# NTT123/vietTTS

Hardware: AMD Instinct MI355X
Metric: audio samples/sec whole-node, HiFi-GAN V1 mel2wave (higher is better)
Workload: dtype bf16; 1 GPU; HiFi-GAN V1 generator, 64 utterances x 1024 mel frames per GPU per step (BASELINE configs[2] shape), bf16; batch_per_gpu=64, frames=1024, parallelism=dp1 utterance-sharded, weights broadcast once, no data-path collective, microbatch=0, streams=0, schedule=engine default: micro-batches of <= 32768 frames on two HIP streams

## Files before the change

viettts_amd/csrc/kernels_bf16_rbg.hip:

```cpp
#include <stdio.h>
#include <string.h>

#include <type_traits>
#include <utility>

#include "bf16_common.h"

namespace vtts {

template <class F, int... I>
__device__ __forceinline__ void static_for(std::integer_sequence<int, I...>, F&& f) {
    (f(std::integral_constant<int, I>{}), ...);
}

constexpr int XCD_MAP_MIN_TILES = 192;

template <int C_, int KS_, int N1_, int WM_, int WN_, int PA_, int MINWG_, int XC_ = C_, int BLK_ = 32>
struct GTile {
    static constexpr int C = C_, KS = KS_, N1 = N1_, WM = WM_, WN = WN_, PA = PA_, MINWG = MINWG_, BLK = BLK_;
    static constexpr int XC = XC_, NXC = C / XC;
    static constexpr int MR16 = C / WM / 16, NR16 = N1 / WN / 16, NH = NR16 / 4;
    static constexpr int KS32 = C / 32, KSX32 = XC / 32;
        static constexpr int LA16 = 3, RA16 = LA16 + 1;
    static_assert(BLK == 32 || BLK == 16, "MFMA block shape");
    static_assert(BLK == 32 || (XC >= 64 && C / WM == 64 && (N1 / WN) % 64 == 0 && (KSX32 % 4 == 0 || (NXC == 1 && 4 % KSX32 == 0)) && 4 % RA16 == 0), "16-block tiles: C >= 64, 64-row wave tiles");
    static constexpr int THREADS = 64 * WM * WN;
    static constexpr int MR = C / WM / 32, NR = N1 / WN / 32;
    static constexpr int H2 = (KS - 1) / 2;
    static constexpr int MAXDIL = 5;
    static constexpr int NT2 = N1 - 2 * H2;
    static constexpr int SPR1 = XC / 8, P1 = XC * 2;
    static constexpr int SPR2 = C / 8, P2 = C * 2;
    static constexpr int ROWSX_MAX = N1 + 2 * H2 * MAXDIL;
    static constexpr int ROWST = N1 + 2 * H2;
    static constexpr int KSTEPS = C / 16;
    static constexpr int KSX = XC / 16;
    static constexpr int NQT = KS * KSTEPS;
    static constexpr int MB = C / 32;
    static constexpr int RA = PA + 1;
    static constexpr bool UNROLL_ALL = (KSX % RA) != 0;
    static constexpr bool WREG = UNROLL_ALL && NXC == 1 && NQT * MR * 4 <= 96;
    static constexpr int XPT = (ROWSX_MAX * SPR1 + THREADS - 1) / THREADS;
    static constexpr size_t CONV_BYTES = (size_t)KS * C * C * 2;
    static_assert(C % (WM * 32) == 0 && N1 % (WN * 32) == 0, "tile/wave mismatch");
    static_assert(C % XC == 0 && (NXC == 1 || !UNROLL_ALL), "channel chunking");
    static_assert(SPR1 == 4 || SPR1 == 8 || SPR1 == 16, "X row pitch 64..256 B");
    static_assert(SPR2 == 4 || SPR2 == 8 || SPR2 == 16 || SPR2 == 32, "xt row pitch 64..512 B");
    static constexpr bool RAWRES = NXC == 1 && C == 32;
    static constexpr int RAW_BYTES = RAWRES ? tile_rows16(N1) * P1 : 0;
    static __host__ __device__ constexpr int tile_bytes(int dil) {
        const int bx = tile_rows16(N1 + 2 * H2 * dil) * P1, bt = tile_rows16(ROWST) * P2;
        return bx > bt ? bx : bt;
    }
    static constexpr bool TAIL = false;
    static constexpr int TAIL_KS = 7, TAIL_H = 3;
    static constexpr int TAIL_BYTES = 0;
    static constexpr bool UP = false;
    static constexpr int OH = 0;
    static int lds_bytes(int dil) { return tile_bytes(dil) + RAW_BYTES; }
    static_assert(tile_rows16(ROWSX_MAX) * P1 + RAW_BYTES <= 80 * 1024 || !RAWRES, "two workgroups per CU");
    static_assert(tile_rows16(ROWSX_MAX) * P1 <= 160 * 1024 && tile_rows16(ROWST) * P2 <= 160 * 1024, "LDS budget");
};

template <class B>
struct GTail : B {
    static constexpr bool TAIL = true;
    static constexpr int TAIL_BYTES = 1024;
    static constexpr int OH = B::TAIL_H;
    static int lds_bytes(int dil) { return B::tile_bytes(dil) + B::RAW_BYTES + TAIL_BYTES; }
    static_assert(B::RAWRES && B::C == 32 && B::WM == 1, "the tail lives on the C = 32 tile with the LDS-resident residual rows");
    static_assert(B::tile_bytes(B::MAXDIL) + B::RAW_BYTES + TAIL_BYTES <= 80 * 1024, "two workgroups per CU");
};

template <class B>
struct GUp : B {
    static constexpr bool UP = true;
    static constexpr int OH = 1;
    static constexpr int UWN = B::WM * B::WN;
    static constexpr int UNR = B::N1 / UWN / 32;
    static constexpr int UMR = B::C / 2 / 32;
    static constexpr int UKS = B::C / 16;
    static constexpr int UP_BYTES = 3 * B::C * B::C * 2;
    static_assert(B::BLK == 16 && !B::RAWRES && !B::TAIL && B::NXC == 1 && (B::C == 128 || B::C == 64), "the stage-ending k = 11 classes (both run 16-blocks)");
    static_assert(B::N1 % (UWN * 32) == 0 && UMR >= 1 && UKS % 2 == 0, "whole 32 x 32 blocks");
    static_assert(B::N1 + 2 <= B::ROWST, "frames t0 - 1 .. t0 + N1 fit the xt tile");
    static_assert(B::tile_bytes(B::MAXDIL) <= 80 * 1024, "two workgroups per CU");
};

template <class T>
__global__ __launch_bounds__(T::THREADS, (T::MINWG * T::THREADS + 255) / 256) void resblock_pair_g_bf16_k(BConvArgs a) {
    constexpr int C = T::C, KS = T::KS, N1 = T::N1, WN = T::WN, PA = T::PA, RA = T::RA;
    constexpr int THREADS = T::THREADS, MR = T::MR, NR = T::NR, H2 = T::H2, NT2 = T::NT2;
    constexpr int SPR1 = T::SPR1, P1 = T::P1, SPR2 = T::SPR2, P2 = T::P2, XC = T::XC, NXC = T::NXC, KSX = T::KSX;
    constexpr int KSTEPS = T::KSTEPS, NQT = T::NQT, MB = T::MB, XPT = T::XPT;
    constexpr int BLK = T::BLK;
    constexpr bool B16 = BLK == 16;
    constexpr int MR16 = T::MR16, NR16 = T::NR16, NH = T::NH;
    static_assert(!B16 || (!T::RAWRES && !T::TAIL && !T::WREG && !T::UNROLL_ALL), "16-block tiles are the rolled-loop C >= 64 tiles");

    extern __shared__ __attribute__((aligned(16))) unsigned char lds[];
    unsigned char* xt = lds;
    [[maybe_unused]] unsigned char* const xraw = lds + (T::RAWRES ? T::tile_bytes(a.dil) : 0);

    const int tid = threadIdx.x;
    const int lane = tid & 63;
    const int wave = tid >> 6;
    const int wm = wave / WN;
    const int wn = wave % WN;
    const int l31 = lane & 31;
    const int lh = lane >> 5;
    const int l15 = lane & 15;
    const int lg = lane >> 4;
    const int b = a.zrev ? (int)(gridDim.z - 1 - blockIdx.z) : (int)blockIdx.z;
    const int Lp = a.L;
    const int L = a.lens ? min(max(a.lens[b], 0) * a.len_mul, a.L) : a.L;
    constexpr int OH = T::OH, TS = NT2 - 2 * OH;
    const bool xmap = (a.L + TS - 1) / TS >= XCD_MAP_MIN_TILES;
    const int nt = (L + TS - 1) / TS, r = (int)((blockIdx.x + b) & 7), lo = (r * nt) >> 3, hi = ((r + 1) * nt) >> 3;
    const int tile = xmap ? lo + (int)(blockIdx.x >> 3) : (int)blockIdx.x;
    if (xmap && tile >= hi) return;
    const int t0 = tile * TS - OH;
    if (t0 + OH >= L) return;
    const int dil = a.dil;
    const int h1 = H2 * dil;
    const int rowsx = N1 + 2 * h1;
    const unsigned short* __restrict__ xg = static_cast<const unsigned short*>(a.x) + (size_t)b * Lp * C;
    [[maybe_unused]] const int wg_lin = blockIdx.z * gridDim.x + blockIdx.x;
    VTTS_TL_ID(a, wg_lin);
    VTTS_TL(a, wg_lin, 0);

    typedef float f32x4 __attribute__((ext_vector_type(4)));
    f32x16 acc[B16 ? 1 : MR][B16 ? 1 : NR];
    f32x16 bblk[B16 ? 1 : MR];
    f32x4 acc16[B16 ? MR16 : 1][B16 ? NR16 : 1];
    f32x4 bblk16[B16 ? MR16 : 1];
    auto load_bias = [&](const float* __restrict__ bias) {
        typedef float f32x8 __attribute__((ext_vector_type(8)));
        if constexpr (B16) {
#pragma unroll
            for (int mr = 0; mr < MR16; ++mr) bblk16[mr] = *reinterpret_cast<const f32x4*>(bias + wm * (C / T::WM) + mr * 16 + 4 * lg);
            return;
        }
#pragma unroll
        for (int mr = 0; mr < MR; ++mr) {
            const float* __restrict__ bp = bias + wm * (C / T::WM) + mr * 32 + 4 * lh;
            const f32x4 q0 = *reinterpret_cast<const f32x4*>(bp), q1 = *reinterpret_cast<const f32x4*>(bp + 8);
            const f32x4 q2 = *reinterpret_cast<const f32x4*>(bp + 16), q3 = *reinterpret_cast<const f32x4*>(bp + 24);
            const f32x8 lo = __builtin_shufflevector(q0, q1, 0, 1, 2, 3, 4, 5, 6, 7), hi = __builtin_shufflevector(q2, q3, 0, 1, 2, 3, 4, 5, 6, 7);
            bblk[mr] = __builtin_shufflevector(lo, hi, 0, 1, 2, 3, 4, 5, 6, 7, 8, 9, 10, 11, 12, 13, 14, 15);
        }
    };
    load_bias(a.bias);
    if constexpr (T::TAIL) {
        float* tw = reinterpret_cast<float*>(lds + T::tile_bytes(dil) + T::RAW_BYTES);
        for (int i = tid; i < T::TAIL_KS * C; i += THREADS) tw[i] = a.tail_wf[i];
    }

    constexpr int NQW = T::WREG ? NQT : 1;
    bf16x8 aw[NQW][MR];
    auto load_w_all = [&](const unsigned char* __restrict__ wconv) {
        if constexpr (T::WREG) {
            const uint4* __restrict__ ap = reinterpret_cast<const uint4*>(wconv) + (size_t)(wm * MR) * 64 + lane;
#pragma unroll
            for (int q = 0; q < NQT; ++q)
#pragma unroll
                for (int mr = 0; mr < MR; ++mr) aw[q][mr] = __builtin_bit_cast(bf16x8, ap[(size_t)(q * MB + mr) * 64]);
        }
    };
    load_w_all(static_cast<const unsigned char*>(a.wp));

    auto stage_x = [&](int xc, auto xb_tag) {
        constexpr int XB = decltype(xb_tag)::value;
        constexpr int RPI = THREADS / SPR1;
        static_assert(THREADS % SPR1 == 0 && RPI % 16 == 0, "a thread's units share their column and their swizzle");
        const int tx0 = t0 - H2 - h1;
        constexpr int RW = 64 / SPR1;
        const int row0 = SPR1 >= 16 ? tid / SPR1 : wave * RW + lane % RW, c = SPR1 >= 16 ? tid % SPR1 : lane / RW;
        auto act2 = [](unsigned u) { return lrelu01_pack(bf16_lo(u), bf16_hi(u)); };
        unsigned char* const lds0 = xt + tile_off<SPR1, BLK>(row0, c);
        [[maybe_unused]] auto keep_raw = [&](int r, int cc, const uint4& raw, bool live) {
            const int rr = r - H2 - h1;
            if (live && rr >= 0 && rr < N1) *reinterpret_cast<uint4*>(xraw + tile_off<SPR1, BLK>(rr, cc)) = raw;
        };
        if (tx0 >= 0 && tx0 + XPT * RPI <= L) {
            const unsigned short* __restrict__ g0 = xg + (size_t)(tx0 + row0) * C + xc * XC + c * 8;
#pragma unroll
            for (int i0 = 0; i0 < XPT; i0 += XB) {
                uint4 v[XB];
#pragma unroll
                for (int i = 0; i < XB; ++i)
                    if (i0 + i < XPT) v[i] = *reinterpret_cast<const uint4*>(g0 + (size_t)(i0 + i) * RPI * C);
#if VTTS_TIMELINE
                if (i0 == 0) {
                    VTTS_TL(a, wg_lin, 7);
                    __builtin_amdgcn_s_waitcnt(0x0f70);
                    VTTS_TL(a, wg_lin, 8);
                }
#endif
                if constexpr (T::RAWRES) {
#pragma unroll
                    for (int i = 0; i < XB; ++i) keep_raw(row0 + (i0 + i) * RPI, c, v[i], i0 + i < XPT);
                }
#pragma unroll
                for (int i = 0; i < XB; ++i) {
                    v[i].x = act2(v[i].x);
                    v[i].y = act2(v[i].y);
                    v[i].z = act2(v[i].z);
                    v[i].w = act2(v[i].w);
                }
#pragma unroll
                for (int i = 0; i < XB; ++i)
                    if (i0 + i < XPT && row0 + (i0 + i) * RPI < rowsx) *reinterpret_cast<uint4*>(lds0 + (i0 + i) * RPI * P1) = v[i];
            }
            return;
        }
#pragma unroll
        for (int i0 = 0; i0 < XPT; i0 += XB) {
            uint4 v[XB];
            bool okx[XB];
#pragma unroll
            for (int i = 0; i < XB; ++i) {
                const int t = tx0 + row0 + (i0 + i) * RPI;
                okx[i] = i0 + i < XPT && row0 + (i0 + i) * RPI < rowsx && t >= 0 && t < L;
                const int tc = t < 0 ? 0 : (t >= L ? L - 1 : t);
                v[i] = *reinterpret_cast<const uint4*>(xg + (size_t)tc * C + xc * XC + c * 8);
            }
#pragma unroll
            for (int i = 0; i < XB; ++i) {
                if (!okx[i]) v[i] = make_uint4(0u, 0u, 0u, 0u);
                if constexpr (T::RAWRES) keep_raw(row0 + (i0 + i) * RPI, c, v[i], i0 + i < XPT);
                v[i].x = act2(v[i].x);
                v[i].y = act2(v[i].y);
                v[i].z = act2(v[i].z);
                v[i].w = act2(v[i].w);
            }
#pragma unroll
            for (int i = 0; i < XB; ++i)
                if (i0 + i < XPT && row0 + (i0 + i) * RPI < rowsx) *reinterpret_cast<uint4*>(lds0 + (i0 + i) * RPI * P1) = v[i];
        }
    };
    stage_x(0, std::integral_constant<int, XPT>{});
    VTTS_TL(a, wg_lin, 9);
    __syncthreads();
    VTTS_TL(a, wg_lin, 1);

    const int rowbase0 = wn * (N1 / WN) + l31;
    auto conv_phase = [&](const unsigned char* __restrict__ wconv, int dl, auto sprb_tag, auto nks_tag, int ks0, auto fresh_tag) {
        constexpr int SPRB = decltype(sprb_tag)::value, PB = SPRB * 16, NKS = decltype(nks_tag)::value;
        constexpr bool FRESH = decltype(fresh_tag)::value;
        constexpr int NSTEPS = KS * NKS;
        const uint4* __restrict__ aptr = reinterpret_cast<const uint4*>(wconv) + ((size_t)ks0 * MB + wm * MR) * 64 + lane;
        bf16x8 af[RA][MR], bf[2][NR];
        auto load_a = [&](int tap, int ks, int slot) {
            const int tc = tap < KS ? tap : KS - 1;
#pragma unroll
            for (int mr = 0; mr < MR; ++mr)
                af[slot][mr] = __builtin_bit_cast(bf16x8, aptr[(size_t)((tc * KSTEPS + ks) * MB + mr) * 64]);
        };
        auto load_b = [&](int tap, int ks, int par) {
#pragma unroll
            for (int nr = 0; nr < NR; ++nr) {
                const int row = rowbase0 + tap * dl + nr * 32;
                bf[par][nr] = *reinterpret_cast<const bf16x8*>(xt + tile_off<SPRB, BLK>(row, ks * 2 + lh));
            }
        };
        auto mfma_step = [&](int slot, int par, bool first) {
#pragma unroll
            for (int mr = 0; mr < MR; ++mr)
#pragma unroll
                for (int nr = 0; nr < NR; ++nr) {
                    acc[mr][nr] = __builtin_amdgcn_mfma_f32_32x32x16_bf16(af[slot][mr], bf[par][nr], first ? bblk[mr] : acc[mr][nr], 0, 0, 0);

                }
        };
        auto pin_step = [&](bool has_b) {
            constexpr int NM = MR * NR;
            const int mem = MR + (has_b ? NR : 0);
            int done = 0;
            for (int i = 0; i < NM; ++i) {
                __builtin_amdgcn_sched_group_barrier(0x008, 1, 0);
                const int upto = (i + 1) * mem / NM;
                for (; done < upto; ++done) {
                    if (done < MR) __builtin_amdgcn_sched_group_barrier(0x020, 1, 0);
                    else __builtin_amdgcn_sched_group_barrier(0x100, 1, 0);
                }
            }
        };
        static_assert(T::UNROLL_ALL || PA <= NKS, "look-ahead within two taps");
#pragma unroll
        for (int s = 0; s < PA; ++s) load_a(s / NKS, s % NKS, s % RA);
        load_b(0, 0, 0);
        __builtin_amdgcn_sched_group_barrier(0x020, MR * PA, 0);
        __builtin_amdgcn_sched_group_barrier(0x100, NR, 0);
        if constexpr (T::UNROLL_ALL) {
#pragma unroll
            for (int s = 0; s < NSTEPS; ++s) {
                load_a((s + PA) / NKS, (s + PA) % NKS, (s + PA) % RA);
                if (s + 1 < NSTEPS) load_b((s + 1) / NKS, (s + 1) % NKS, (s + 1) & 1);
                mfma_step(s % RA, s & 1, FRESH && s == 0);
                pin_step(s + 1 < NSTEPS);
            }
        } else {
            constexpr int UB = NKS < 8 ? NKS : 8;
            static_assert(T::UNROLL_ALL || (UB % RA == 0 && UB % 2 == 0 && NKS % UB == 0), "ring slot / B parity must be compile-time in the block loop");
            typedef unsigned u32x4_t __attribute__((ext_vector_type(4)));
            const auto rs_w = __builtin_amdgcn_make_buffer_rsrc(const_cast<unsigned char*>(wconv), 0, (int)T::CONV_BYTES, 0x00020000);
            const unsigned a_voff = (unsigned)((wm * MR) * 64 + lane) * 16;
            auto load_a2 = [&](int sa, int slot) {
                const int sc = sa < NSTEPS ? sa : NSTEPS - 1;
                const int tap = sc / NKS, ks = sc - tap * NKS;
                const int soff = ((tap * KSTEPS + ks0 + ks) * MB) * 1024;
#pragma unroll
                for (int mr = 0; mr < MR; ++mr) {
                    const u32x4_t v = __builtin_amdgcn_raw_buffer_load_b128(rs_w, a_voff + mr * 1024, soff, 0);
                    af[slot][mr] = __builtin_bit_cast(bf16x8, v);
                }
            };
            auto tap_terms = [&](int tap, unsigned& tapaddr, unsigned& xs) {
                const int row = rowbase0 + tap * dl;
                if constexpr (SPRB >= 16) {
                    tapaddr = (unsigned)row * PB;
                    xs = (unsigned)(swz_of<SPRB>(row) ^ lh) << 4;
                } else {
                    tapaddr = (unsigned)tile_off<SPRB, BLK>(row, lh);
                    xs = 0;
                }
            };
            auto load_b2 = [&](unsigned tapaddr, unsigned xs, int ks, int par) {
                const unsigned addr = SPRB >= 16 ? tapaddr + (xs ^ (unsigned)(ks << 5)) : tapaddr + (unsigned)(ks << 9);
#pragma unroll
                for (int nr = 0; nr < NR; ++nr) bf[par][nr] = *reinterpret_cast<const bf16x8*>(xt + addr + nr * 32 * PB);
            };
            auto block = [&](int s0, auto first_tag) {
                const int tap = s0 / NKS, ksb = s0 - tap * NKS;
                unsigned ta, xs, tn, xn;
                tap_terms(tap, ta, xs);
                const bool wrap = ksb + UB >= NKS;
                const int tapn = tap + 1 < KS ? tap + 1 : KS - 1;
                tap_terms(wrap ? tapn : tap, tn, xn);
                const int ksn = wrap ? 0 : ksb + UB;
#pragma unroll
                for (int i = 0; i < UB; ++i) {
                    load_a2(s0 + i + PA, (i + PA) % RA);
                    if (i + 1 < UB) load_b2(ta, xs, ksb + i + 1, (i + 1) & 1);
                    else load_b2(tn, xn, ksn, (i + 1) & 1);
                    mfma_step(i % RA, i & 1, decltype(first_tag)::value && i == 0);
                    pin_step(true);
                }
            };
            block(0, std::integral_constant<bool, FRESH>{});
#pragma nounroll
            for (int s0 = UB; s0 < NSTEPS; s0 += UB) block(s0, std::false_type{});
        }
    };

    auto conv_phase_wreg = [&](int dl, auto sprb_tag) {
        constexpr int SPRB = decltype(sprb_tag)::value;
        bf16x8 bf[2][NR];
        auto load_b = [&](int q, int par) {
            const int tap = q / KSTEPS, ks = q % KSTEPS;
#pragma unroll
            for (int nr = 0; nr < NR; ++nr) bf[par][nr] = *reinterpret_cast<const bf16x8*>(xt + tile_off<SPRB, BLK>(rowbase0 + tap * dl + nr * 32, ks * 2 + lh));
        };
        load_b(0, 0);
        __builtin_amdgcn_sched_group_barrier(0x100, NR, 0);
#pragma unroll
        for (int q = 0; q < NQT; ++q) {
            if (q + 1 < NQT) load_b(q + 1, (q + 1) & 1);
#pragma unroll
            for (int mr = 0; mr < MR; ++mr)
#pragma unroll
                for (int nr = 0; nr < NR; ++nr)
                    acc[mr][nr] = __builtin_amdgcn_mfma_f32_32x32x16_bf16(aw[q < NQW ? q : 0][mr], bf[q & 1][nr], q == 0 ? bblk[mr] : acc[mr][nr], 0, 0, 0);
            for (int i = 0; i < MR * NR; ++i) {
                __builtin_amdgcn_sched_group_barrier(0x008, 1, 0);
                if (q + 1 < NQT && i < NR) __builtin_amdgcn_sched_group_barrier(0x100, 1, 0);
            }
        }
    };


    const int rowbase16 = wn * (N1 / WN) + l15;
    auto conv_phase16 = [&](const unsigned char* __restrict__ wconv, int dl, auto sprb_tag, auto nks_tag, int ks0, auto fresh_tag) {
        constexpr int SPRB = decltype(sprb_tag)::value, PB = SPRB * 16, NKS = decltype(nks_tag)::value;
        constexpr bool FRESH = decltype(fresh_tag)::value;
        constexpr int NSTEPS = KS * NKS, LA = T::LA16, RA = T::RA16, UB = 4, APU = MR16 / NH;
        constexpr int REM = NSTEPS % UB;
        static_assert((NKS % UB == 0 || UB % NKS == 0) && UB % RA == 0 && (UB * NH) % 2 == 0, "ring slot / B parity must be compile-time in the block loop");
        const auto rs_w = __builtin_amdgcn_make_buffer_rsrc(const_cast<unsigned char*>(wconv), 0, (int)T::CONV_BYTES, 0x00020000);
        const unsigned a_voff = (unsigned)((wm * MR16) * 64 + lane) * 16;
        bf16x8 af[RA][MR16], bf[2][4];
        auto load_a = [&](int sa, auto h_tag, auto slot_tag) {
            constexpr int h = decltype(h_tag)::value, slot = decltype(slot_tag)::value;
            const int sc = sa < NSTEPS ? sa : NSTEPS - 1;
            const int tap = sc / NKS, ks = sc - tap * NKS;
            const int soff = ((tap * T::KS32 + ks0 + ks) * (C / 16)) * 1024;
#pragma unroll
            for (int m = h * APU; m < (h + 1) * APU; ++m) af[slot][m] = __builtin_bit_cast(bf16x8, __builtin_amdgcn_raw_buffer_load_b128(rs_w, a_voff + m * 1024, soff, 0));
        };
        auto tap_terms = [&](int tap, unsigned& tapaddr, unsigned& xs) {
            const int row = rowbase16 + tap * dl;
            if constexpr (SPRB >= 16) {
                tapaddr = (unsigned)row * PB;
                xs = (unsigned)(swz_of<SPRB, 16>(row) ^ lg) << 4;
            } else {
                tapaddr = (unsigned)tile_off<SPRB, BLK>(row, lg);
                xs = 0;
            }
        };
        auto load_b = [&](unsigned tapaddr, unsigned xs, int ks, int h, auto par_tag) {
            const unsigned addr = SPRB >= 16 ? tapaddr + (xs ^ (unsigned)(ks << 6)) : tapaddr + (unsigned)(ks << 10);
#pragma unroll
            for (int nr = 0; nr < 4; ++nr) bf[decltype(par_tag)::value][nr] = *reinterpret_cast<const bf16x8*>(xt + addr + (4 * h + nr) * 16 * PB);
        };
        auto pin_unit = [&](auto nds_tag, auto nvm_tag) {
            constexpr int NDS = decltype(nds_tag)::value, NVM = decltype(nvm_tag)::value;
            int done = 0;
#pragma unroll
            for (int i = 0; i < 16; ++i) {
                __builtin_amdgcn_sched_group_barrier(0x008, 1, 0);
                const int upto = (i + 1) * (NDS + NVM) / 16;
#pragma unroll
                for (; done < upto; ++done) {
                    if (done < NDS) __builtin_amdgcn_sched_group_barrier(0x100, 1, 0);
                    else __builtin_amdgcn_sched_group_barrier(0x020, 1, 0);
                }
            }
        };
        unsigned ta0, xs0;
        tap_terms(0, ta0, xs0);
        static_for(std::make_integer_sequence<int, LA * NH>{}, [&](auto v) {
            constexpr int s = decltype(v)::value / NH, h = decltype(v)::value % NH;
            load_a(s, std::integral_constant<int, h>{}, std::integral_constant<int, s % RA>{});
        });
        load_b(ta0, xs0, 0, 0, std::integral_constant<int, 0>{});
        __builtin_amdgcn_sched_group_barrier(0x020, MR16 * LA, 0);
        __builtin_amdgcn_sched_group_barrier(0x100, 4, 0);
        auto block = [&](int s0, auto nu_tag) {
            constexpr int NU = decltype(nu_tag)::value, NT = NKS >= UB ? 1 : (NU + NKS - 1) / NKS;
            constexpr bool PEEL = NU < UB;
            const int tap = s0 / NKS, ksb = s0 - tap * NKS;
            unsigned ta[NT], xs[NT], tn, xn;
#pragma unroll
            for (int t = 0; t < NT; ++t) tap_terms(tap + t, ta[t], xs[t]);
            const bool wrap = ksb + UB >= NKS;
            const int tapn = tap + NT < KS ? tap + NT : KS - 1;
            tap_terms(wrap ? tapn : tap, tn, xn);
            const int ksn = wrap ? 0 : ksb + UB;
            static_for(std::make_integer_sequence<int, NU * NH>{}, [&](auto v) {
                constexpr int u = decltype(v)::value, i = u / NH, h = u % NH;
                constexpr int ti = NKS >= UB ? 0 : i / NKS, ki = i - ti * NKS;
                constexpr int tj = NKS >= UB ? 0 : (i + 1) / NKS, kj = i + 1 - tj * NKS;
                constexpr bool last = h + 1 == NH && i + 1 == NU;
                if constexpr (!PEEL) load_a(s0 + i + LA, std::integral_constant<int, h>{}, std::integral_constant<int, (i + LA) % RA>{});
                constexpr auto par = std::integral_constant<int, (u + 1) & 1>{};
                if constexpr (h + 1 < NH) load_b(ta[ti], xs[ti], ksb + ki, h + 1, par);
                else if constexpr (i + 1 < NU) load_b(ta[tj], xs[tj], ksb + kj, 0, par);
                else if constexpr (!PEEL) load_b(tn, xn, ksn, 0, par);
#pragma unroll
                for (int nr = 0; nr < 4; ++nr)
#pragma unroll
                    for (int mr = 0; mr < MR16; ++mr)
                        acc16[mr][4 * h + nr] = __builtin_amdgcn_mfma_f32_16x16x32_bf16(af[i % RA][mr], bf[u & 1][nr], acc16[mr][4 * h + nr], 0, 0, 0);
                pin_unit(std::integral_constant<int, PEEL && last ? 0 : 4>{}, std::integral_constant<int, PEEL ? 0 : APU>{});
            });
        };
        if constexpr (FRESH) {
#pragma unroll
            for (int mr = 0; mr < MR16; ++mr)
#pragma unroll
                for (int nr = 0; nr < NR16; ++nr) acc16[mr][nr] = bblk16[mr];
        }
#pragma nounroll
        for (int s0 = 0; s0 < NSTEPS - REM; s0 += UB) block(s0, std::integral_constant<int, UB>{});
        if constexpr (REM != 0) block(NSTEPS - REM, std::integral_constant<int, REM>{});
    };

#pragma unroll
    for (int xc = 0; xc < NXC; ++xc) {
        if (xc > 0) {
            __syncthreads();
            stage_x(xc, std::integral_constant<int, 4>{});
            __syncthreads();
        }
        if constexpr (B16) {
            if (xc == 0) conv_phase16(static_cast<const unsigned char*>(a.wp), dil, std::integral_constant<int, SPR1>{}, std::integral_constant<int, T::KSX32>{}, 0, std::true_type{});
            else conv_phase16(static_cast<const unsigned char*>(a.wp), dil, std::integral_constant<int, SPR1>{}, std::integral_constant<int, T::KSX32>{}, xc * T::KSX32, std::false_type{});
        } else if constexpr (T::WREG)
            conv_phase_wreg(dil, std::integral_constant<int, SPR1>{});
        else if (xc == 0)
            conv_phase(static_cast<const unsigned char*>(a.wp), dil, std::integral_constant<int, SPR1>{}, std::integral_constant<int, KSX>{}, 0, std::true_type{});
        else
            conv_phase(static_cast<const unsigned char*>(a.wp), dil, std::integral_constant<int, SPR1>{}, std::integral_constant<int, KSX>{}, xc * KSX, std::false_type{});
    }
    VTTS_TL(a, wg_lin, 2);
    load_w_all(static_cast<const unsigned char*>(a.wp) + T::CONV_BYTES);
    __syncthreads();


    load_bias(a.bias + C);
    [[maybe_unused]] const int col16 = wn * (N1 / WN) + 16 * (lg & 1) + l15;
    {
        if constexpr (B16) {
#pragma unroll
            for (int mr = 0; mr < MR16; ++mr) {
                const int cb = wm * (C / T::WM) + mr * 16;
#pragma unroll
                for (int j = 0; j < NR16 / 2; ++j) {
                    const int tp = t0 - H2 + wn * (N1 / WN) + 32 * j + l15, tq = tp + 16;
                    unsigned p0 = lrelu01_pack(acc16[mr][2 * j][0], acc16[mr][2 * j][1]);
                    unsigned p1 = lrelu01_pack(acc16[mr][2 * j][2], acc16[mr][2 * j][3]);
                    unsigned q0 = lrelu01_pack(acc16[mr][2 * j + 1][0], acc16[mr][2 * j + 1][1]);
                    unsigned q1 = lrelu01_pack(acc16[mr][2 * j + 1][2], acc16[mr][2 * j + 1][3]);
                    if (!(tp >= 0 && tp < L)) p0 = p1 = 0u;
                    if (!(tq >= 0 && tq < L)) q0 = q1 = 0u;
                    swap_pair16(p0, q0);
                    swap_pair16(p1, q1);
                    *reinterpret_cast<uint4*>(xt + tile_off<SPR2, BLK>(col16 + 32 * j, (cb >> 3) + (lg >> 1))) = make_uint4(p0, p1, q0, q1);
                }
            }
        } else {
#pragma unroll
        for (int mr = 0; mr < MR; ++mr) {
#pragma unroll
            for (int p = 0; p < 2; ++p) {
                const int cb = wm * (C / T::WM) + mr * 32 + 16 * p;
#pragma unroll
                for (int nr = 0; nr < NR; ++nr) {
                    const int row = wn * (N1 / WN) + nr * 32 + l31;
                    const int tt = t0 - H2 + row;
                    const bool ok = tt >= 0 && tt < L;
                    const int r0 = 8 * p;
                    unsigned p0 = lrelu01_pack(acc[mr][nr][r0 + 0], acc[mr][nr][r0 + 1]);
                    unsigned p1 = lrelu01_pack(acc[mr][nr][r0 + 2], acc[mr][nr][r0 + 3]);
                    unsigned q0 = lrelu01_pack(acc[mr][nr][r0 + 4], acc[mr][nr][r0 + 5]);
                    unsigned q1 = lrelu01_pack(acc[mr][nr][r0 + 6], acc[mr][nr][r0 + 7]);
                    if (!ok) p0 = p1 = q0 = q1 = 0u;
                    swap_pair(p0, q0);
                    swap_pair(p1, q1);
                    const int slot = (cb >> 3) + lh;
                    *reinterpret_cast<uint4*>(xt + tile_off<SPR2, BLK>(row, slot)) = make_uint4(p0, p1, q0, q1);
                }
            }
        }
        }
        for (int u = tid; u < 2 * H2 * SPR2; u += THREADS) {
            const int row = N1 + u % (2 * H2), c = u / (2 * H2);
            *reinterpret_cast<uint4*>(xt + tile_off<SPR2, BLK>(row, c)) = make_uint4(0u, 0u, 0u, 0u);
        }
    }
    __syncthreads();
    VTTS_TL(a, wg_lin, 3);

    if constexpr (B16)
        conv_phase16(static_cast<const unsigned char*>(a.wp) + T::CONV_BYTES, 1, std::integral_constant<int, SPR2>{}, std::integral_constant<int, T::KS32>{}, 0, std::true_type{});
    else if constexpr (T::WREG)
        conv_phase_wreg(1, std::integral_constant<int, SPR2>{});
    else
        conv_phase(static_cast<const unsigned char*>(a.wp) + T::CONV_BYTES, 1, std::integral_constant<int, SPR2>{}, std::integral_constant<int, KSTEPS>{}, 0, std::true_type{});
    VTTS_TL(a, wg_lin, 4);

    {
        const float s_out = a.slope_out;
        const float dv = a.div;
        const float rdv = mrf_recip(dv);
        unsigned short* __restrict__ yg = static_cast<unsigned short*>(a.y) + (size_t)b * Lp * C;
        auto add_rows = [&](const unsigned short* __restrict__ src) {
            if constexpr (B16) {
                uint4 rv[MR16][NR16 / 2];
#pragma unroll
                for (int mr = 0; mr < MR16; ++mr)
#pragma unroll
                    for (int j = 0; j < NR16 / 2; ++j) {
                        const int t = t0 + col16 + 32 * j;
                        const int tc = t < 0 ? 0 : (t < L ? t : L - 1);
                        rv[mr][j] = *reinterpret_cast<const uint4*>(src + (size_t)tc * C + wm * (C / T::WM) + mr * 16 + 8 * (lg >> 1));
                    }
#pragma unroll
                for (int mr = 0; mr < MR16; ++mr)
#pragma unroll
                    for (int j = 0; j < NR16 / 2; ++j) {
                        uint4 r = rv[mr][j];
                        swap_pair16(r.x, r.z);
                        swap_pair16(r.y, r.w);
                        f32x4& ap = acc16[mr][2 * j];
                        f32x4& aq = acc16[mr][2 * j + 1];
                        ap[0] = vadd_raw(bf16_lo(r.x), ap[0]); ap[1] = vadd_raw(bf16_hi(r.x), ap[1]);
                        ap[2] = vadd_raw(bf16_lo(r.y), ap[2]); ap[3] = vadd_raw(bf16_hi(r.y), ap[3]);
                        aq[0] = vadd_raw(bf16_lo(r.z), aq[0]); aq[1] = vadd_raw(bf16_hi(r.z), aq[1]);
                        aq[2] = vadd_raw(bf16_lo(r.w), aq[2]); aq[3] = vadd_raw(bf16_hi(r.w), aq[3]);
                    }
            } else {
            uint4 rv[MR][2][NR];
#pragma unroll
            for (int mr = 0; mr < MR; ++mr)
#pragma unroll
                for (int p = 0; p < 2; ++p)
#pragma unroll
                    for (int nr = 0; nr < NR; ++nr) {
                        const int t = t0 + wn * (N1 / WN) + nr * 32 + l31;
                        const int tc = t < 0 ? 0 : (t < L ? t : L - 1);
                        rv[mr][p][nr] = *reinterpret_cast<const uint4*>(src + (size_t)tc * C + wm * (C / T::WM) + mr * 32 + 16 * p + 8 * lh);
                    }
#if VTTS_TIMELINE
            VTTS_TL(a, wg_lin, 10);
            __builtin_amdgcn_s_waitcnt(0x0f70);
            VTTS_TL(a, wg_lin, 11);
#endif
#pragma unroll
            for (int mr = 0; mr < MR; ++mr)
#pragma unroll
                for (int p = 0; p < 2; ++p)
#pragma unroll
                    for (int nr = 0; nr < NR; ++nr) {
                        uint4 r = rv[mr][p][nr];
                        swap_pair(r.x, r.z);
                        swap_pair(r.y, r.w);
                        const int r0 = 8 * p;
                        acc[mr][nr][r0 + 0] = vadd_raw(bf16_lo(r.x), acc[mr][nr][r0 + 0]); acc[mr][nr][r0 + 1] = vadd_raw(bf16_hi(r.x), acc[mr][nr][r0 + 1]);
                        acc[mr][nr][r0 + 2] = vadd_raw(bf16_lo(r.y), acc[mr][nr][r0 + 2]); acc[mr][nr][r0 + 3] = vadd_raw(bf16_hi(r.y), acc[mr][nr][r0 + 3]);
                        acc[mr][nr][r0 + 4] = vadd_raw(bf16_lo(r.z), acc[mr][nr][r0 + 4]); acc[mr][nr][r0 + 5] = vadd_raw(bf16_hi(r.z), acc[mr][nr][r0 + 5]);
                        acc[mr][nr][r0 + 6] = vadd_raw(bf16_lo(r.w), acc[mr][nr][r0 + 6]); acc[mr][nr][r0 + 7] = vadd_raw(bf16_hi(r.w), acc[mr][nr][r0 + 7]);
                    }
            }
        };
        if constexpr (T::RAWRES) {
#pragma unroll
            for (int mr = 0; mr < MR; ++mr)
#pragma unroll
                for (int p = 0; p < 2; ++p)
#pragma unroll
                    for (int nr = 0; nr < NR; ++nr) {
                        const int col = wn * (N1 / WN) + nr * 32 + l31;
                        uint4 r = *reinterpret_cast<const uint4*>(xraw + tile_off<SPR1, BLK>(col, (wm * (C / T::WM) + mr * 32 + 16 * p) / 8 + lh));
                        swap_pair(r.x, r.z);
                        swap_pair(r.y, r.w);
                        const int r0 = 8 * p;
                        acc[mr][nr][r0 + 0] = vadd_raw(bf16_lo(r.x), acc[mr][nr][r0 + 0]); acc[mr][nr][r0 + 1] = vadd_raw(bf16_hi(r.x), acc[mr][nr][r0 + 1]);
                        acc[mr][nr][r0 + 2] = vadd_raw(bf16_lo(r.y), acc[mr][nr][r0 + 2]); acc[mr][nr][r0 + 3] = vadd_raw(bf16_hi(r.y), acc[mr][nr][r0 + 3]);
                        acc[mr][nr][r0 + 4] = vadd_raw(bf16_lo(r.z), acc[mr][nr][r0 + 4]); acc[mr][nr][r0 + 5] = vadd_raw(bf16_hi(r.z), acc[mr][nr][r0 + 5]);
                        acc[mr][nr][r0 + 6] = vadd_raw(bf16_lo(r.w), acc[mr][nr][r0 + 6]); acc[mr][nr][r0 + 7] = vadd_raw(bf16_hi(r.w), acc[mr][nr][r0 + 7]);
                    }
        } else {
            add_rows(xg);
        }
        if (a.acc_add != 0) add_rows(yg);
        VTTS_TL(a, wg_lin, 12);
        if constexpr (T::UP) {
            __syncthreads();
            VTTS_TL(a, wg_lin, 5);
        }
        if constexpr (B16) {
#pragma unroll
            for (int mr = 0; mr < MR16; ++mr) {
                const int cb = wm * (C / T::WM) + mr * 16;
#pragma unroll
                for (int j = 0; j < NR16 / 2; ++j) {
                    const int row = col16 + 32 * j;
                    const int t = t0 + row;
                    const bool ok = (T::UP || row < NT2) && t >= 0 && t < L;
                    float v[8];
#pragma unroll
                    for (int e = 0; e < 4; ++e) {
                        v[e] = acc16[mr][2 * j][e];
                        v[4 + e] = acc16[mr][2 * j + 1][e];
                    }
                    if (dv != 1.0f) {
#pragma unroll
                        for (int e = 0; e < 8; ++e) v[e] = v[e] * rdv;
                    }
                    if (s_out != 1.0f) {
#pragma unroll
                        for (int e = 0; e < 8; ++e) v[e] = lrelu_f(v[e], s_out);
                    }
                    unsigned p0 = pack_bf16x2(v[0], v[1]), p1 = pack_bf16x2(v[2], v[3]);
                    unsigned q0 = pack_bf16x2(v[4], v[5]), q1 = pack_bf16x2(v[6], v[7]);
                    swap_pair16(p0, q0);
                    swap_pair16(p1, q1);
                    if constexpr (T::UP) {
                        const uint4 o = ok ? make_uint4(p0, p1, q0, q1) : make_uint4(0u, 0u, 0u, 0u);
                        *reinterpret_cast<uint4*>(xt + tile_off<SPR2, 32>(row, (cb >> 3) + (lg >> 1))) = o;
                    } else {
                        if (ok) *reinterpret_cast<uint4*>(yg + (size_t)t * C + cb + 8 * (lg >> 1)) = make_uint4(p0, p1, q0, q1);
                    }
                }
            }
        } else {
#pragma unroll
        for (int mr = 0; mr < MR; ++mr) {
#pragma unroll
            for (int p = 0; p < 2; ++p) {
                const int cb = wm * (C / T::WM) + mr * 32 + 16 * p;
#pragma unroll
                for (int nr = 0; nr < NR; ++nr) {
                    const int row = wn * (N1 / WN) + nr * 32 + l31;
                    const int t = t0 + row;
                    const bool ok = row < NT2 && t >= 0 && t < L;
                    float v[8];
#pragma unroll
                    for (int e = 0; e < 8; ++e) v[e] = acc[mr][nr][8 * p + e];
                    if (dv != 1.0f) {
#pragma unroll
                        for (int e = 0; e < 8; ++e) v[e] = v[e] * rdv;
                    }
                    if (s_out != 1.0f) {
#pragma unroll
                        for (int e = 0; e < 8; ++e) v[e] = lrelu_f(v[e], s_out);
                    }
                    unsigned p0 = pack_bf16x2(v[0], v[1]), p1 = pack_bf16x2(v[2], v[3]);
                    unsigned q0 = pack_bf16x2(v[4], v[5]), q1 = pack_bf16x2(v[6], v[7]);
                    swap_pair(p0, q0);
                    swap_pair(p1, q1);
                    if constexpr (T::TAIL) {
                        const uint4 o = ok ? make_uint4(p0, p1, q0, q1) : make_uint4(0u, 0u, 0u, 0u);
                        if (row < NT2) *reinterpret_cast<uint4*>(xraw + tile_off<SPR1, BLK>(row, (cb >> 3) + lh)) = o;
                    } else {
                        if (ok) *reinterpret_cast<uint4*>(yg + (size_t)t * C + cb + 8 * lh) = make_uint4(p0, p1, q0, q1);
                    }
                }
            }
        }
        }
    }
    if constexpr (T::UP) {
        constexpr int UNR = T::UNR, UMR = T::UMR, UKS = T::UKS, UMB = C / 32, NQ = 2 * UKS, UPA = 3, URA = UPA + 1;
        typedef unsigned u32x4_t __attribute__((ext_vector_type(4)));
        const auto rs_u = __builtin_amdgcn_make_buffer_rsrc(const_cast<void*>(a.up_wp), 0, T::UP_BYTES, 0x00020000);
        const unsigned u_voff = (unsigned)lane * 16;
        const int ucol = wave * (N1 / T::UWN) + l31;
        unsigned short* __restrict__ zg = static_cast<unsigned short*>(a.up_y) + (size_t)b * Lp * C;
        f32x16 uacc[UMR][UNR], ub[2][UMR];
        bf16x8 uaf[URA][UMR], ubf[2][UNR];
#pragma unroll
        for (int c = 0; c < 2; ++c)
#pragma unroll
            for (int mr = 0; mr < UMR; ++mr) {
                typedef float f32x8 __attribute__((ext_vector_type(8)));
                const float* __restrict__ bp = a.up_bias + c * (C / 2) + mr * 32 + 4 * lh;
                const f32x4 q0 = *reinterpret_cast<const f32x4*>(bp), q1 = *reinterpret_cast<const f32x4*>(bp + 8);
                const f32x4 q2 = *reinterpret_cast<const f32x4*>(bp + 16), q3 = *reinterpret_cast<const f32x4*>(bp + 24);
                const f32x8 lo = __builtin_shufflevector(q0, q1, 0, 1, 2, 3, 4, 5, 6, 7), hi = __builtin_shufflevector(q2, q3, 0, 1, 2, 3, 4, 5, 6, 7);
                ub[c][mr] = __builtin_shufflevector(lo, hi, 0, 1, 2, 3, 4, 5, 6, 7, 8, 9, 10, 11, 12, 13, 14, 15);
            }
        auto uload_a = [&](auto g_tag) {
            constexpr int g = decltype(g_tag)::value, c = g / NQ, s = g % NQ, f = c + s / UKS, ks = s % UKS;
            constexpr int soff = ((f * UKS + ks) * UMB + c * UMR) * 1024;
#pragma unroll
            for (int mr = 0; mr < UMR; ++mr) uaf[g % URA][mr] = __builtin_bit_cast(bf16x8, __builtin_amdgcn_raw_buffer_load_b128(rs_u, u_voff + mr * 1024, soff, 0));
        };
        auto uload_b = [&](auto g_tag) {
            constexpr int g = decltype(g_tag)::value, c = g / NQ, s = g % NQ, f = c + s / UKS, ks = s % UKS;
#pragma unroll
            for (int nr = 0; nr < UNR; ++nr) ubf[g & 1][nr] = *reinterpret_cast<const bf16x8*>(xt + tile_off<SPR2, 32>(ucol + 32 * nr + f, 2 * ks + lh));
        };
        static_for(std::make_integer_sequence<int, UPA>{}, uload_a);
        __syncthreads();
        VTTS_TL(a, wg_lin, 13);
        uload_b(std::integral_constant<int, 0>{});
        static_for(std::make_integer_sequence<int, 2 * NQ>{}, [&](auto g_tag) {
            constexpr int g = decltype(g_tag)::value, c = g / NQ, s = g % NQ;
            constexpr bool more_a = g + UPA < 2 * NQ, more_b = g + 1 < 2 * NQ;
            if constexpr (more_a) uload_a(std::integral_constant<int, g + UPA>{});
            if constexpr (more_b) uload_b(std::integral_constant<int, g + 1>{});
#pragma unroll
            for (int mr = 0; mr < UMR; ++mr)
#pragma unroll
                for (int nr = 0; nr < UNR; ++nr)
                    uacc[mr][nr] = __builtin_amdgcn_mfma_f32_32x32x16_bf16(uaf[g % URA][mr], ubf[g & 1][nr], s == 0 ? ub[c][mr] : uacc[mr][nr], 0, 0, 0);
            pin_loads<UMR * UNR, more_a ? UMR : 0, more_b ? UNR : 0>();
            if constexpr (s + 1 == NQ) {
#pragma unroll
                for (int mr = 0; mr < UMR; ++mr)
#pragma unroll
                    for (int p = 0; p < 2; ++p) {
                        const int rb = c * (C / 2) + mr * 32 + 16 * p;
#pragma unroll
                        for (int nr = 0; nr < UNR; ++nr) {
                            const int n = ucol + 32 * nr, q = t0 + OH + n;
                            unsigned p0 = pack_bf16x2(uacc[mr][nr][8 * p + 0], uacc[mr][nr][8 * p + 1]), p1 = pack_bf16x2(uacc[mr][nr][8 * p + 2], uacc[mr][nr][8 * p + 3]);
                            unsigned q0 = pack_bf16x2(uacc[mr][nr][8 * p + 4], uacc[mr][nr][8 * p + 5]), q1 = pack_bf16x2(uacc[mr][nr][8 * p + 6], uacc[mr][nr][8 * p + 7]);
                            swap_pair(p0, q0);
                            swap_pair(p1, q1);
                            if (n < TS && q < L) *reinterpret_cast<uint4*>(zg + (size_t)q * C + rb + 8 * lh) = make_uint4(p0, p1, q0, q1);
                        }
                    }
            }
        });
    }
    if constexpr (T::TAIL) {
        __syncthreads();
        const float* tw = reinterpret_cast<const float*>(lds + T::tile_bytes(dil) + T::RAW_BYTES);
        const float tb = a.tail_bias[0];
        for (int n = tid; n < TS; n += THREADS) {
            const int t = t0 + T::TAIL_H + n;
            if (t >= L) break;
            float accp = 0.f;
#pragma unroll
            for (int j = 0; j < T::TAIL_KS; ++j) {
#pragma unroll
                for (int c = 0; c < SPR1; ++c) {
                    const uint4 v = *reinterpret_cast<const uint4*>(xraw + tile_off<SPR1, BLK>(n + j, c));
                    const float* w = tw + j * C + c * 8;
                    accp = fmaf(w[0], bf16_lo(v.x), accp); accp = fmaf(w[1], bf16_hi(v.x), accp);
                    accp = fmaf(w[2], bf16_lo(v.y), accp); accp = fmaf(w[3], bf16_hi(v.y), accp);
                    accp = fmaf(w[4], bf16_lo(v.z), accp); accp = fmaf(w[5], bf16_hi(v.z), accp);
                    accp = fmaf(w[6], bf16_lo(v.w), accp); accp = fmaf(w[7], bf16_hi(v.w), accp);
                }
            }
            a.tail_wav[(size_t)b * Lp + t] = tanhf(accp + tb);
        }
    }
    VTTS_TL(a, wg_lin, 6);
}

#ifndef VTTS_EXP_LDS_PAD
#define VTTS_EXP_LDS_PAD 0
#endif
#ifndef VTTS_G64_N1
#define VTTS_G64_N1 512
#define VTTS_G64_WG 2
#endif
#ifndef VTTS_G32_N1
#define VTTS_G32_N1 512
#define VTTS_G32_WG 2
#endif
#ifndef VTTS_G128K3_N1
#define VTTS_G128K3_N1 256
#define VTTS_G128K3_WG 2
#endif
constexpr int g_mfma_blk(int C, int KS) {
    return C == 256 ? (KS == 3 ? 16 : KS == 7 ? 32 : 16)
         : C == 128 ? (KS == 3 ? 16 : KS == 7 ? 16 : 16)
         : C == 64  ? (KS == 3 ? 32 : KS == 7 ? 16 : 16)
                    : 32;
}
template <int KS> using G128 = GTile<128, KS, KS == 3 ? VTTS_G128K3_N1 : 256, 2, 2, 3, KS == 3 ? VTTS_G128K3_WG : 2, 128, g_mfma_blk(128, KS)>;
template <int KS> using G64 = GTile<64, KS, VTTS_G64_N1, 1, 4, 3, VTTS_G64_WG, 64, g_mfma_blk(64, KS)>;
#ifndef VTTS_G32_PA
#define VTTS_G32_PA 3
#endif
template <int KS> using G32 = GTile<32, KS, VTTS_G32_N1, 1, 4, VTTS_G32_PA, VTTS_G32_WG>;
template <int KS> using G256 = GTile<256, KS, 128, 4, 1, 3, 2, 128, g_mfma_blk(256, KS)>;
template <int KS> using G256S = GTile<256, KS, 64, 4, 1, 3, 2, 128, g_mfma_blk(256, KS)>;
template <int KS> using G128S = GTile<128, KS, 128, 2, 2, 3, 2, 128, g_mfma_blk(128, KS)>;
template <int KS> using G64S = GTile<64, KS, 256, 1, 4, 3, 2, 64, g_mfma_blk(64, KS)>;
template <int KS> using G32S = GTile<32, KS, 256, 1, 4, 3, 2>;
constexpr long G_MIN_WGS = 384;
template <class T>
static hipError_t launch_g(const BConvArgs& a, hipStream_t s) {
    static DynLdsOnce once;
    if (hipError_t e = set_max_dynamic_lds(reinterpret_cast<const void*>(&resblock_pair_g_bf16_k<T>), T::lds_bytes(T::MAXDIL) + VTTS_EXP_LDS_PAD, once); e != hipSuccess) return e;
    if (a.dil < 1 || a.dil > T::MAXDIL) return hipErrorInvalidValue;
    constexpr int TS = T::NT2 - 2 * T::OH;
    dim3 grid((a.L + TS - 1) / TS, 1, a.B);
    if ((int)grid.x >= XCD_MAP_MIN_TILES) grid.x = (grid.x + 7) / 8 * 8;
    hipLaunchKernelGGL(resblock_pair_g_bf16_k<T>, grid, dim3(T::THREADS), T::lds_bytes(a.dil) + VTTS_EXP_LDS_PAD, s, a);
    return hipGetLastError();
}

template <template <int> class TT>
static hipError_t launch_g_ks(const BConvArgs& a, int K, hipStream_t s) {
    switch (K) {
        case 3: return launch_g<TT<3>>(a, s);
        case 7: return launch_g<TT<7>>(a, s);
        case 11: return launch_g<TT<11>>(a, s);
    }
    return hipErrorInvalidValue;
}

hipError_t launch_pair_g_bf16(int C, int K, const BConvArgs& a, hipStream_t s) {
    auto narrow = [&](int nt2) { return a.tile_pref == 2 || (a.tile_pref != 1 && (long)((a.L + nt2 - 1) / nt2) * a.B < G_MIN_WGS); };
    if (a.up_y) {
        if (K != 11 || a.tail_wav) return hipErrorInvalidValue;
        if (C == 128) return narrow(G128<11>::NT2) ? launch_g<GUp<G128S<11>>>(a, s) : launch_g<GUp<G128<11>>>(a, s);
        if (C == 64) return narrow(G64<11>::NT2) ? launch_g<GUp<G64S<11>>>(a, s) : launch_g<GUp<G64<11>>>(a, s);
        return hipErrorInvalidValue;
    }
    switch (C) {
        case 256: return narrow(G256<11>::NT2) ? launch_g_ks<G256S>(a, K, s) : launch_g_ks<G256>(a, K, s);
        case 128: return narrow(G128<11>::NT2) ? launch_g_ks<G128S>(a, K, s) : launch_g_ks<G128>(a, K, s);
        case 64: return narrow(G64<11>::NT2) ? launch_g_ks<G64S>(a, K, s) : launch_g_ks<G64>(a, K, s);
        case 32:
            if (a.tail_wav) {
                if (K != 11) return hipErrorInvalidValue;
                return narrow(G32<11>::NT2) ? launch_g<GTail<G32S<11>>>(a, s) : launch_g<GTail<G32<11>>>(a, s);
            }
            return narrow(G32<11>::NT2) ? launch_g_ks<G32S>(a, K, s) : launch_g_ks<G32>(a, K, s);
    }
    return hipErrorInvalidValue;
}

bool pair_tail_bf16_supported(int C, int K, int post_cin, int post_cout, int post_k) { return C == 32 && K == 11 && post_cin == 32 && post_cout == 1 && post_k == 7; }

bool pair_up_bf16_supported(int C, int K, int up_cls, int up_cin, int up_cout, int up_k, int up_stride) {
    return K == 11 && ((C == 128 && up_cls == BCLS_UP2) || (C == 64 && up_cls == BCLS_UP3)) && up_cin == C && 2 * up_cout == C && up_k == 4 && up_stride == 2;
}

BPackGeom pair_g_pack_geom(int C, int K) { return BPackGeom{C, C, C, K, C, 1}; }

int pair_g_mfma_blk(int C, int K) { return g_mfma_blk(C, K); }

void pair_g_pack(const float* Wc, int C, int K, unsigned short* out) {
    if (g_mfma_blk(C, K) == 16) pair_g_pack16(Wc, C, K, out);
    else bf16_pack(Wc, C, pair_g_pack_geom(C, K), out);
}

const char* pair_g_kernel_name(int C, int K) {
    static thread_local char buf[96];
    snprintf(buf, sizeof(buf), "resblock_pair_g_bf16_k<GTile<%d, %d,", C, K);
    return buf;
}

bool pair_bf16_supported(int C, int K, int dil) {
    return (C == 256 || C == 128 || C == 64 || C == 32) && (K == 3 || K == 7 || K == 11) && dil >= 1 && dil <= 5;
}

}
```

Baseline: 448.4 million samples/s.

## Compute tail conv two samples per thread with weights from scalar memory

The final 7-tap output conv no longer stages its weights in LDS. It reads them through the constant address space into scalar registers, and each thread computes two adjacent output samples so input rows are shared across both. Row loads and weight loads for the next tap are software-pipelined, with schedule barriers, against the FMAs of the current tap. It also adds timeline probes under VTTS_TIMELINE. The change cuts LDS traffic and redundant row reads in the tail, at the cost of higher VGPR pressure and a new assumption that one pass of threads covers the whole tile.

```diff
diff --git a/viettts_amd/csrc/kernels_bf16_rbg.hip b/viettts_amd/csrc/kernels_bf16_rbg.hip
--- a/viettts_amd/csrc/kernels_bf16_rbg.hip
+++ b/viettts_amd/csrc/kernels_bf16_rbg.hip
@@ -54,7 +54,6 @@
     }
     static constexpr bool TAIL = false;
     static constexpr int TAIL_KS = 7, TAIL_H = 3;
-    static constexpr int TAIL_BYTES = 0;
     static constexpr bool UP = false;
     static constexpr int OH = 0;
     static int lds_bytes(int dil) { return tile_bytes(dil) + RAW_BYTES; }
@@ -65,11 +64,10 @@
 template <class B>
 struct GTail : B {
     static constexpr bool TAIL = true;
-    static constexpr int TAIL_BYTES = 1024;
     static constexpr int OH = B::TAIL_H;
-    static int lds_bytes(int dil) { return B::tile_bytes(dil) + B::RAW_BYTES + TAIL_BYTES; }
+    static constexpr int SPT = 2;
     static_assert(B::RAWRES && B::C == 32 && B::WM == 1, "the tail lives on the C = 32 tile with the LDS-resident residual rows");
-    static_assert(B::tile_bytes(B::MAXDIL) + B::RAW_BYTES + TAIL_BYTES <= 80 * 1024, "two workgroups per CU");
+    static_assert((B::NT2 - 2 * OH) % SPT == 0 && B::NT2 - 2 * OH <= SPT * B::THREADS, "a tile's samples are whole groups, one per thread");
 };
 
 template <class B>
@@ -151,10 +149,6 @@
         }
     };
     load_bias(a.bias);
-    if constexpr (T::TAIL) {
-        float* tw = reinterpret_cast<float*>(lds + T::tile_bytes(dil) + T::RAW_BYTES);
-        for (int i = tid; i < T::TAIL_KS * C; i += THREADS) tw[i] = a.tail_wf[i];
-    }
 
     constexpr int NQW = T::WREG ? NQT : 1;
     bf16x8 aw[NQW][MR];
@@ -757,6 +751,10 @@
         __syncthreads();
         VTTS_TL(a, wg_lin, 13);
         uload_b(std::integral_constant<int, 0>{});
+#if VTTS_TIMELINE
+        __builtin_amdgcn_s_waitcnt(0x0070);
+        VTTS_TL(a, wg_lin, 14);
+#endif
         static_for(std::make_integer_sequence<int, 2 * NQ>{}, [&](auto g_tag) {
             constexpr int g = decltype(g_tag)::value, c = g / NQ, s = g % NQ;
             constexpr bool more_a = g + UPA < 2 * NQ, more_b = g + 1 < 2 * NQ;
@@ -769,6 +767,7 @@
                     uacc[mr][nr] = __builtin_amdgcn_mfma_f32_32x32x16_bf16(uaf[g % URA][mr], ubf[g & 1][nr], s == 0 ? ub[c][mr] : uacc[mr][nr], 0, 0, 0);
             pin_loads<UMR * UNR, more_a ? UMR : 0, more_b ? UNR : 0>();
             if constexpr (s + 1 == NQ) {
+                if constexpr (c == 0) VTTS_TL(a, wg_lin, 10);
 #pragma unroll
                 for (int mr = 0; mr < UMR; ++mr)
 #pragma unroll
@@ -784,30 +783,66 @@
                             if (n < TS && q < L) *reinterpret_cast<uint4*>(zg + (size_t)q * C + rb + 8 * lh) = make_uint4(p0, p1, q0, q1);
                         }
                     }
+                if constexpr (c == 0) VTTS_TL(a, wg_lin, 11);
             }
         });
     }
     if constexpr (T::TAIL) {
+        constexpr int SPT = T::SPT;
         __syncthreads();
-        const float* tw = reinterpret_cast<const float*>(lds + T::tile_bytes(dil) + T::RAW_BYTES);
+        VTTS_TL(a, wg_lin, 5);
+        typedef const __attribute__((address_space(4))) float* cfloat_p;
+        const cfloat_p tw = (cfloat_p)a.tail_wf;
         const float tb = a.tail_bias[0];
-        for (int n = tid; n < TS; n += THREADS) {
-            const int t = t0 + T::TAIL_H + n;
-            if (t >= L) break;
-            float accp = 0.f;
+        const int n = SPT * tid, t = t0 + T::TAIL_H + n;
+        if (n < TS && t < L) {
+            constexpr int NROWS = T::TAIL_KS + SPT - 1;
+            uint4 pk[NROWS][SPR1];
+            float x[NROWS][C], w[T::TAIL_KS][C], accp[SPT];
+            auto read_row = [&](int r) {
+#pragma unroll
+                for (int c = 0; c < SPR1; ++c) pk[r][c] = *reinterpret_cast<const uint4*>(xraw + tile_off<SPR1, BLK>(n + r, c));
+            };
+            auto unpack_row = [&](int r) {
+#pragma unroll
+                for (int c = 0; c < SPR1; ++c) {
+                    const uint4 v = pk[r][c];
+                    x[r][8 * c + 0] = bf16_lo(v.x); x[r][8 * c + 1] = bf16_hi(v.x); x[r][8 * c + 2] = bf16_lo(v.y); x[r][8 * c + 3] = bf16_hi(v.y);
+                    x[r][8 * c + 4] = bf16_lo(v.z); x[r][8 * c + 5] = bf16_hi(v.z); x[r][8 * c + 6] = bf16_lo(v.w); x[r][8 * c + 7] = bf16_hi(v.w);
+                }
+            };
+            int woff = 0;
+            auto load_w = [&](int j) {
+#pragma unroll
+                for (int i = 0; i < C; ++i) w[j][i] = tw[j * C + woff + i];
+            };
+            load_w(0);
+#pragma unroll
+            for (int r = 0; r < SPT; ++r) read_row(r);
+#pragma unroll
+            for (int r = 0; r < SPT; ++r) unpack_row(r);
+#pragma unroll
+            for (int s = 0; s < SPT; ++s) accp[s] = 0.f;
 #pragma unroll
             for (int j = 0; j < T::TAIL_KS; ++j) {
-#pragma unroll
-                for (int c = 0; c < SPR1; ++c) {
-                    const uint4 v = *reinterpret_cast<const uint4*>(xraw + tile_off<SPR1, BLK>(n + j, c));
-                    const float* w = tw + j * C + c * 8;
-                    accp = fmaf(w[0], bf16_lo(v.x), accp); accp = fmaf(w[1], bf16_hi(v.x), accp);
-                    accp = fmaf(w[2], bf16_lo(v.y), accp); accp = fmaf(w[3], bf16_hi(v.y), accp);
-                    accp = fmaf(w[4], bf16_lo(v.z), accp); accp = fmaf(w[5], bf16_hi(v.z), accp);
-                    accp = fmaf(w[6], bf16_lo(v.w), accp); accp = fmaf(w[7], bf16_hi(v.w), accp);
-                }
-            }
-            a.tail_wav[(size_t)b * Lp + t] = tanhf(accp + tb);
+                if (j + 1 < T::TAIL_KS) {
+                    asm volatile("" : "+s"(woff) : : "memory");
+                    load_w(j + 1);
+                    read_row(j + SPT);
+                }
+#pragma unroll
+                for (int s = 0; s < SPT; ++s)
+#pragma unroll
+                    for (int i = 0; i < C; ++i) accp[s] = fmaf(w[j][i], x[j + s][i], accp[s]);
+                if (j + 1 < T::TAIL_KS) unpack_row(j + SPT);
+#pragma unroll
+                for (int s = 0; s < SPT; ++s) asm volatile("" : "+v"(accp[s]));
+                __builtin_amdgcn_sched_barrier(0);
+            }
+            VTTS_TL(a, wg_lin, 14);
+#pragma unroll
+            for (int s = 0; s < SPT; ++s)
+                if (t + s < L) a.tail_wav[(size_t)b * Lp + t + s] = tanhf(accp[s] + tb);
         }
     }
     VTTS_TL(a, wg_lin, 6);
```

Result: no change. 449.6 million samples/s, median of 6 (+0.3%).
